# FT-Autonomous/ft_grandprix

Measured on AMD Instinct MI355X. Metric: env-steps/sec (4096 envs, 1080-ray LiDAR) at 1/2/4/8 MI355X; HBM roofline %, higher is better.
Workload: dtype f32 rays + f64 state

## Files before the change

ft_grandprix_amd/csrc/ftgp_api.hip:

```cpp
#include <dlfcn.h>
#include <math.h>
#include <cmath>
#include <stdarg.h>
#include <stdio.h>
#include <stdlib.h>
#include <string.h>

#include <algorithm>
#include <memory>
#include <string>
#include <type_traits>
#include <utility>
#include <vector>

#include <hip/hip_ext.h>
#include "ftgp_kernels.hip"

namespace {

thread_local char g_err[512] = "";

int fail(int code, const char* fmt, const char* a = "")
{
    snprintf(g_err, sizeof g_err, fmt, a);
    return code;
}

int failf(int code, const char* fmt, ...)
{
    va_list ap;
    va_start(ap, fmt);
    vsnprintf(g_err, sizeof g_err, fmt, ap);
    va_end(ap);
    return code;
}

int name_track(int code, int k)
{
    const std::string m(g_err);
// ... 366 lines not shown
        return FTGP_ERR_ARG;
    }
    if (sw.verbose)
        fprintf(stderr, "ftgp_create: %d cars x %d waves per workgroup, %d B of LDS (cap %d)\n", cpb, wpb, lds_layout(P, cpb, wpb), lds_cap);
    return 0;
}

void plan_fan(const FtgpConfig& cfg, std::vector<float>& ray, std::vector<double>& fan)
{
    const int R = cfg.n_rays;
    ray.assign((size_t)pad16(sizeof(float) * 2 * (size_t)R) / sizeof(float), 0.0f);
    fan.assign(2 * (size_t)R, 0.0);
    for (int j = 0; j < R; ++j) {
        const double phi = ((360.0 / (double)R) * (double)j - 90.0) * (M_PI / 180.0);
        fan[2 * (size_t)j] = cfg.fan_dirs ? cfg.fan_dirs[2 * (size_t)j] : sin(phi);
        fan[2 * (size_t)j + 1] = cfg.fan_dirs ? cfg.fan_dirs[2 * (size_t)j + 1] : -cos(phi);
        ray[2 * (size_t)j] = (float)fan[2 * (size_t)j]; ray[2 * (size_t)j + 1] = (float)fan[2 * (size_t)j + 1];
        if (!cfg.fan_dirs && R % 2 == 0 && j >= R / 2) {
            ray[2 * (size_t)j] = -ray[2 * (size_t)(j - R / 2)]; ray[2 * (size_t)j + 1] = -ray[2 * (size_t)(j - R / 2) + 1];
        }
    }
}

void plan_task_order(const FtgpConfig& cfg, const std::vector<float>& ray, const Switches& sw, DeviceParams& P)
{
    const int R = cfg.n_rays, halfR = R / 2;
    bool sym = R % 2 == 0 && !sw.no_pairs;
    for (int j = 0; sym && j < halfR; ++j)
        sym = ray[2 * (size_t)(j + halfR)] == -ray[2 * (size_t)j] && ray[2 * (size_t)(j + halfR) + 1] == -ray[2 * (size_t)j + 1] &&
              std::signbit(ray[2 * (size_t)(j + halfR)]) != std::signbit(ray[2 * (size_t)j]) && std::signbit(ray[2 * (size_t)(j + halfR) + 1]) != std::signbit(ray[2 * (size_t)j + 1]);
    std::vector<int> tasks;
    if (!sym) for (int j0 = 0; j0 < R; j0 += FTGP_WAVE) tasks.push_back(j0);
    else {
        int j0 = 0;
        for (; j0 + FTGP_WAVE <= halfR; j0 += FTGP_WAVE) tasks.push_back(j0 | (1 << 16));
        if (j0 < halfR) tasks.push_back(j0 | ((halfR - j0 <= FTGP_WAVE / 2 ? 2 : 1) << 16));
    }
    std::vector<std::pair<double, int>> key;
    for (int t : tasks) {
        const double mid = std::min((double)R - 1.0, (double)(t & 0xffff) + 31.5);
        key.push_back({ sw.group_order_plain ? 0.0 : -fabs(cos(2.0 * M_PI * mid / (double)R)), t });
    }
    std::stable_sort(key.begin(), key.end(), [](const std::pair<double, int>& a, const std::pair<double, int>& b) { return a.first < b.first; });
    const int tail = sw.pair_tail;
    std::vector<int> order;
    for (size_t k = 0; k < key.size(); ++k) {
        const int t = key[k].second;
        if ((t >> 16) == 1 && (int)(key.size() - k) <= tail) { order.push_back(t & 0xffff); order.push_back((t & 0xffff) + halfR); }
        else order.push_back(t);
    }
    P.tasks_per_car = (int)order.size();
    for (size_t k = 0; k < order.size(); ++k) P.group_order[k] = order[k];
    const double gamma = 32.0 * (2.0 * M_PI / (double)R) + 0.021;
// ... 7 lines not shown
    const int cpb = P.cars_per_block, ntasks = cpb * P.tasks_per_car, R = P.n_rays, halfR = R / 2;
    if (P.tasks_per_car > 256 || R > 0x4000) return fail(FTGP_ERR_ARG, "internal: the task table's fields are too narrow for this fan%s");
    tt.assign(2 * 4 * (size_t)ntasks, 0);
    auto wclass = [&](int first, int lim) {
        const int last = std::min(first + FTGP_WAVE, lim) - 1, lo = P.eighth, hi = R - P.eighth;
        if (last < lo || first >= hi || lo >= hi) return 0;
        return (first >= lo && last < hi) ? 1 : 2;
    };
    for (int g = 0; g < ntasks; ++g) {
        const int kidx = g / cpb, c = g % cpb, ent = P.group_order[kidx], j0 = ent & 0xffff, kind = ent >> 16;
        const int w0 = kind == 2 ? 2 : wclass(j0, kind == 1 ? halfR : R), w1 = kind == 1 ? wclass(j0 + halfR, R) : 0;
        const uint32_t plain = (uint32_t)j0 | (uint32_t)kind << 14 | (uint32_t)c << 16;
        int32_t* a = &tt[4 * (size_t)g];
        int32_t* b = &tt[4 * (size_t)(ntasks + g)];
        a[0] = (int32_t)(plain | (uint32_t)w0 << 20 | (uint32_t)w1 << 22 | (uint32_t)(j0 == 0 ? 1 : 0) << 24);
        b[0] = (int32_t)plain;
        a[1] = b[1] = c * (int)sizeof(LidarFrame) | kidx << 16;
        a[2] = b[2] = c * P.ranges_stride * 4;
        a[3] = b[3] = 4 * (c * P.win_floats + (P.eighth & 3) - P.eighth);
    }
    return 0;
}

void plan_window_table(const Switches& sw, const std::vector<int32_t>& tt, DeviceParams& P, std::vector<int32_t>& tw)
{
    const int cpb = P.cars_per_block, R = P.n_rays, halfR = R / 2;
    tw.clear();
    P.win_tasks_per_car = 0;
    if (sw.scan_every_step) {
        if (sw.verbose) fprintf(stderr, "ftgp_create: FTGP_SCAN_EVERY_STEP: every step of a launch sweeps and stores every ray\n");
        return;
    }
    auto live = [&](int j) { return j == 0 || (j >= P.eighth && j < R - P.eighth); };
    std::vector<std::pair<int, uint32_t>> list;
    for (int k = 0; k < P.tasks_per_car; ++k) {
        uint32_t x = (uint32_t)tt[4 * (size_t)k * cpb];
        const int j0 = x & 0x3fff, kind = (x >> 14) & 3;
        int n[2] = { 0, 0 }, l[2] = { 0, 0 };
        for (int lane = 0; lane < FTGP_WAVE; ++lane) {
            int j; bool mine;
            if (kind == 2) { j = j0 + (lane & 31) + (lane >= 32 ? halfR : 0); mine = (lane & 31) < halfR - j0; }
            else { j = j0 + lane; mine = j < (kind == 1 ? halfR : R); }
            if (!mine) continue;
            ++n[0]; l[0] += live(j) ? 1 : 0;
            if (kind == 1) { ++n[1]; l[1] += live(j + halfR) ? 1 : 0; }
        }
        if (l[0] + l[1] == 0) continue;
        if (kind == 1 && n[0] == FTGP_WAVE && (l[0] == 0 || l[1] == 0)) {
            if (l[0] == 0) { x = (uint32_t)(j0 + halfR) | ((x >> 22) & 3u) << 20 | 1u << 26; n[0] = n[1]; l[0] = l[1]; }
            else x &= ~(3u << 14 | 3u << 22);
            n[1] = l[1] = 0;
        }
        if (l[0] + l[1] < n[0] + n[1]) x |= 1u << 25;
        list.push_back({ k, x });
    }
    P.win_tasks_per_car = (int)list.size();
    const int ntasks = cpb * P.win_tasks_per_car;
    tw.assign(4 * (size_t)ntasks, 0);
    for (int g = 0; g < ntasks; ++g) {
        const int c = g % cpb, kidx = list[(size_t)(g / cpb)].first;
        const int32_t* a = &tt[4 * ((size_t)kidx * cpb + c)];
        int32_t* w = &tw[4 * (size_t)g];
        w[0] = (int32_t)(list[(size_t)(g / cpb)].second | (uint32_t)c << 16);
        w[1] = a[1]; w[2] = a[2]; w[3] = a[3];
    }
    if (sw.verbose) fprintf(stderr, "ftgp_create: %d of them on the window-only steps of a launch\n", P.win_tasks_per_car);
}

double track_diagonal(const FtgpTrack& t) { return hypot((double)t.width * t.px_size_x, (double)t.height * t.px_size_y); }

void plan_vehicle(const DeviceParams& P, double diag, const Switches& sw, std::vector<unsigned char>& img)
{
    const FtgpVehicle& v = P.veh;
    img.assign((size_t)pad16(sizeof(VehLds)), 0);
    VehLds vl; memset(&vl, 0, sizeof vl);
    vl.v = P.veh; for (int i = 0; i < 4; ++i) vl.wheel_load[i] = P.wheel_load[i];
    const double cx = std::max(fabs(v.box_xmin), fabs(v.box_xmax)), cy = std::max(fabs(v.box_ymin), fabs(v.box_ymax));
    const double rmax = std::max(sqrt(cx * cx + cy * cy), sqrt(v.lidar_x * v.lidar_x + v.lidar_y * v.lidar_y) + v.lidar_ring_radius);
    vl.cull_radius = (float)(1.1 * rmax);
    {
        const double r = v.lidar_ring_radius;
        const double need = r > 0.0 ? 5.0 * ldexp(1.0, -24) * diag * diag / (2.0 * r) : 0.0;
        const double have = std::min(std::min(v.lidar_x - r - v.box_xmin, v.box_xmax - (v.lidar_x + r)), std::min(v.lidar_y - r - v.box_ymin, v.box_ymax - (v.lidar_y + r)));
        vl.puck_in_box = (have >= need && !sw.puck_test) ? 1 : 0;
        if (sw.verbose)
            fprintf(stderr, "ftgp_create: inter-vehicle rays test %s (the puck lies %.4f inside the box, %.4f needed on a map of diagonal %.2f)\n",
                    vl.puck_in_box ? "the box only" : "the box and the puck's circle", have, need, diag);
// ... 66 lines not shown
    P.veh = cfg.vehicle;
    {
        const double wtot = v.mass * v.gravity;
        if (v.kind == FTGP_VEHICLE_TRICYCLE) {
            const double a_f = v.wheel_x[2], a_r = -0.5 * (v.wheel_x[0] + v.wheel_x[1]);
            P.wheel_load[0] = P.wheel_load[1] = 0.5 * (wtot * (a_f / (a_f + a_r)));
            P.wheel_load[2] = wtot * (a_r / (a_f + a_r)); P.wheel_load[3] = 0.0;
        } else {
            const double a_f = 0.5 * (v.wheel_x[0] + v.wheel_x[1]), a_r = -0.5 * (v.wheel_x[2] + v.wheel_x[3]);
            P.wheel_load[0] = P.wheel_load[1] = 0.5 * (wtot * (a_r / (a_f + a_r)));
            P.wheel_load[2] = P.wheel_load[3] = 0.5 * (wtot * (a_f / (a_f + a_r)));
        }
    }
    P.eighth = (int)((double)cfg.n_rays / 8.0);
    const double tiny = (double)1.401298464e-45f;
    P.cover_kmax = std::max(1, std::max(cover_count_host(0.24, P.rpp, tiny), cover_count_host(0.12, P.rpp, tiny)));
    P.win_floats = ((P.eighth & 3) + (cfg.n_rays - 2 * P.eighth) + 1 + 3) & ~3;
    P.n_cu = n_cu;
    if ((cfg.n_rays + FTGP_WAVE - 1) / FTGP_WAVE > FTGP_MAX_GROUPS) return fail(FTGP_ERR_ARG, "n_rays above 16384 is not supported%s");
    if (int rc = plan_shape(P, sw)) return rc;
    plan_fan(cfg, pl.ray, pl.fan);
    plan_task_order(cfg, pl.ray, sw, P);
    if (int rc = plan_task_table(P, pl.tasks)) return rc;
    plan_window_table(sw, pl.tasks, P, pl.tasks_win);
    {
        const size_t stride = (size_t)P.cover_kmax + 1, padded = (size_t)pad16(sizeof(float) * stride) / sizeof(float);
        pl.cover.assign(stride + padded + 4, 0.0f);
        build_cover_table(0.12, cfg.n_rays, P.cover_kmax, pl.cover.data());
        build_cover_table(0.06, cfg.n_rays, P.cover_kmax, pl.cover.data() + stride);
    }
    double diag = 0.0;
    pl.env_track.clear();
    for (int t = 0; t < n_tracks; ++t) {
        Plan::Track& k = pl.tracks[(size_t)t];
        k.P = P;
        plan_track_params(cfg, tracks[t], k.P);
        plan_track_tables(tracks[t], k.P, k.tab, k.spawn);
        k.clear.assign(2 * FTGP_PATH_POINTS, 0.0);
        ftgp_start_table(tracks[t], k.spawn.data(), k.clear.data());
        k.path.assign(tracks[t].path, tracks[t].path + 2 * FTGP_PATH_POINTS);
        diag = std::max(diag, track_diagonal(tracks[t]));
        pl.env_track.insert(pl.env_track.end(), (size_t)envs_per_track[t], t);
    }
    plan_vehicle(P, diag, sw, pl.veh);
    plan_workgroups(P.cars_per_block, cfg.cars_per_env, envs_per_track, n_tracks, sw.track_order, pl.wg);
    pl.n_wg = (int)pl.wg.size() / 4;
    if (sw.verbose)
// ... 2001 lines not shown
```

ft_grandprix_amd/csrc/ftgp_device.h:

```cpp
#pragma once
#include <hip/hip_runtime.h>
#include <stdint.h>
#include <stddef.h>
#include "../../include/ftgp.h"
#include "ftgp_march.h"
#include "ftgp_spawn.h"
#include "ftgp_net.h"
#include "ftgp_frame.h"
#include "ftgp_rival.h"

#define FTGP_WAVE 64
#define FTGP_MAX_GROUPS 256
#define FTGP_MAX_CARS_PER_BLOCK 16

struct alignas(16) CarCore {
    double x, y, qw, qz;
    double vx, vy, wz;
    double qs, qsd;
    double w[4];
    double u_speed, u_steer;
    double last_steer;
    double dist2;
    int32_t completion, laps, offset, n_times;
    int32_t good_start, finished, off_track, delta;
// ... 56 lines not shown
    const uint16_t* field;
    const uint32_t* bits;
    const uint32_t* nearbits;
    const void* veh_dev;
    const double* path;
    const double* spawn;
    const float* ray_dir;
    const float* cover_thr;
    CarState* cars;
    float* ranges;
    int64_t* steps;
    double* wg_metrics;
    unsigned int* wg_ticket;
    double* metrics_dev;
    double* metrics_host;
    double* wg_metrics_host;
    alignas(16) int32_t sector_tab[FTGP_SECTORS][4];
    FtgpVehicle veh;
    double wheel_load[4];
    const unsigned char* stage_img;
    int32_t stage_cover, reserved3;
    int32_t car_policy[FTGP_MAX_CARS_PER_BLOCK];
    int32_t group_order[FTGP_MAX_GROUPS];
    const int32_t* task_tab;
};

#define FTGP_PARAMS_BYTES ((sizeof(DeviceParams) + 15) & ~(size_t)15)

struct VehLds {
    FtgpVehicle v;
    double wheel_load[4];
    float cull_radius;
    int32_t puck_in_box;
    float box_xmin_f, box_xmax_f, box_ymin_f, box_ymax_f, lidar_x_f, lidar_y_f, ring_radius_f, pad_f;
};

enum { kDynMass = 0, kDynIzz, kDynFriction, kDynTireDamping, kDynThrottleKv, kDynThrottleForceLimit, kDynSteerKp, kDynSteerDamping, kDynWheelLoad };
template <class PP> __host__ __device__ inline double* dyn_table(PP p) { return reinterpret_cast<double*>(((uint64_t)p->dyn_table_hi << 32) | (uint64_t)p->dyn_table_lo); }
template <class PP> __host__ __device__ inline unsigned long long* dyn_rejected(PP p) { return reinterpret_cast<unsigned long long*>(dyn_table(p) + (size_t)p->n_cars * FTGP_DYN_RECORD); }
#define FTGP_DYN_BYTES(n_cars) ((size_t)(n_cars) * FTGP_DYN_RECORD * sizeof(double) + 16)
struct DynArgs {
    double base[FTGP_DYN_DOUBLES];
    double gravity, load_k[4];
    int32_t load_half[4];
    int32_t init, pad;
    const double* rows;
    const uint8_t* env_mask;
    const uint8_t* env_mask_or;
// ... 80 lines not shown
```

ft_grandprix_amd/csrc/ftgp_kernels.hip:

```cpp
#include "ftgp_device.h"

struct Force { double fx, fy, tz; };
struct Dyn { double x, y, qw, qz, vx, vy, wz, qs, qsd, w[4]; };
static_assert(sizeof(Dyn) == 104 && offsetof(CarCore, w) == offsetof(Dyn, w) && offsetof(CarCore, qsd) == offsetof(Dyn, qsd), "Dyn must mirror the head of CarCore");
#define FTGP_FORCE_TERMS 11

struct Lds {
    const VehLds* veh;
    const double* path;
    const float2* ray;
    CarCore* cars;
    LidarFrame* frame;
    PairCull* pairs;
    int64_t* steps;
    float* scan;
    int* list;
    int* pool;
    Force* terms;
    double* wnew;
    Dyn* next;
    Force* mates;
    const float* cover;
    unsigned char* mmask;
};
// ... 226 lines not shown
        "s_branch L_march_done_%=\n"
        "L_march_fix0_%=:\n\t"
        FTGP_MARCH_FIX("v_mov_b32_e32 %[f], 0\n\t", "%[mx]", "%[my]", "L_march_arrive0_%=")
        "L_march_fix1_%=:\n\t"
        FTGP_MARCH_FIX("v_cndmask_b32_e64 %[f], %[mx], %[my], %[stepx]\n\t", "%[nx]", "%[ny]", "L_march_arrive1_%=")
        "L_march_fix2_%=:\n\t"
        FTGP_MARCH_FIX("v_cndmask_b32_e64 %[f], %[nx], %[ny], %[stepx]\n\t", "%[mx]", "%[my]", "L_march_arrive2_%=")
        "L_march_done_%=:\n\t"
        "s_mov_b64 exec, %[ex0]\n\t"
        "v_min_f32_e32 %[s], %[a], %[b]"
        : [s] "=&v"(s), [w] "=&v"(w), [mx] "=&v"(mx), [my] "=&v"(my), [nx] "=&v"(nx), [ny] "=&v"(ny),
          [a] "=&v"(a), [b] "=&v"(b), [c] "=&v"(c), [d] "=&v"(d), [e] "=&v"(e), [f] "=&v"(f), [h] "=&v"(h), [i] "=&v"(i),
          [gu] "=&v"(gu), [gv] "=&v"(gv), [cx] "=&v"(cx), [cy] "=&v"(cy),
          [stepx] "=&s"(stepx), [sv] "=&s"(sv), [sq] "=&s"(sq), [ex0] "=&s"(ex0)
        : [pu] "v"(pu), [pv] "v"(pv), [ivx] "v"(ivx), [ivy] "v"(ivy), [du] "v"(du), [dv] "v"(dv),
          [base] "v"(base), [ax] "v"(ax), [ay] "v"(ay), [thr] "s"(thr), [field] "s"(field)
        : "vcc", "scc", "memory");
#undef FTGP_MARCH_BODY
#undef FTGP_MARCH_MOVE
#undef FTGP_MARCH_ARRIVE
#undef FTGP_MARCH_FIX
}

template <bool MULTI, bool WINDOW>
__device__ __forceinline__ void lidar_groups(const DeviceParams& P, ScalarParams G, const Lds& L, const LidarFrame* frames, const PairCull* pairs, const unsigned char* mmask,
                                             float* scan_rows, int* pool, int ncars_here, int ci0, bool scan_lds, bool second_half STAMP_ARG)
{
    typedef __attribute__((address_space(1))) float* global_f32;
    typedef __attribute__((address_space(1))) unsigned char* global_u8w;
    struct alignas(16) Task { int32_t x, y, z, w; };
    typedef const __attribute__((address_space(4))) Task* ScalarTasks;
    constexpr bool window_only = WINDOW;
    const int full_tasks = G->cars_per_block * G->tasks_per_car;
    const int R = G->n_rays, half = R >> 1, ntasks = window_only ? G->cars_per_block * G->win_tasks_per_car : full_tasks;
    const int W = G->width, H = G->height, fstride = G->fstride;
    const uint32_t plane256 = G->plane256;
    const int eighth = G->eighth, win_floats = G->win_floats;
    const float isx = G->inv_px_x_f, isy = G->inv_px_y_f, thr = 0.5f - G->snap_eps, nsf = G->slice_factor;
    const float r0 = sgpr(L.veh->ring_radius_f);
    const void* field = G->field;
    const ScalarTasks tasks = (ScalarTasks)G->task_tab + (window_only ? 2 * full_tasks : scan_lds ? 0 : full_tasks);
    const global_u8w ranges = (global_u8w)((global_f32)G->ranges + (size_t)ci0 * G->ranges_stride);
    const int mmask_stride = G->mmask_stride;
    const int lane = lane_here();
    const bool all_safe = sgpr(pool[4]) == 0;
    sweep_priority(second_half);
    for (;;) {
        STAMP(ta);
        int g = 0;
        if (lane == 0) g = atomicAdd(pool, 1);
        g = __builtin_amdgcn_readfirstlane(g);
        if (g >= ntasks) break;
        Task task; { const uint32_t gu = (uint32_t)g; task.x = tasks[gu].x; task.y = tasks[gu].y; task.z = tasks[gu].z; task.w = tasks[gu].w; }
        const int j0 = task.x & 0x3fff, kind = (task.x >> 14) & 3, c = (task.x >> 16) & 15;
        int j; bool mine;
        if (kind == 2) { j = j0 + (lane & 31) + (lane >= 32 ? half : 0); mine = (lane & 31) < half - j0; }
        else { j = j0 + lane; mine = j < (kind == 1 ? half : R); }
        mine = mine && c < ncars_here;
        bool first = mine;
        if (WINDOW && (task.x & (1 << 25))) {
            asm volatile("");
            first = mine && (j == 0 || (unsigned)(j - eighth) < (unsigned)(R - 2 * eighth));
            mine = first || (kind == 1 && mine && (unsigned)(j + half - eighth) < (unsigned)(R - 2 * eighth));
        }
        const LidarFrame* frame = reinterpret_cast<const LidarFrame*>(reinterpret_cast<const unsigned char*>(frames) + (task.y & 0xffff));
        FtgpRay ray;
        float du, dv, dxw, dyw, opu, opv;
        uint32_t sector;
        asm volatile("" : "=v"(du), "=v"(dv), "=v"(dxw), "=v"(dyw), "=v"(opu), "=v"(opv), "=v"(sector));
        auto finish = [&](bool active, int pass) {
            if (!active) return;
            uint32_t w;
            STAMP(tb);
            march_all(ray.s, w, opu, opv, ray.ivx, ray.ivy, du, dv, ray.base, ray.ax, ray.ay, thr, field);
            STAMP(tc); STAMP_ADD(10, tc - tb); STAMP_ADD(9, 1);
            float r = (w == 0u) ? fabsf(ray.s) : ray.result;
            if (MULTI && FTGP_DIAG_RUN_MATES) {
                const PairCull* mates = pairs + c * FTGP_PAIR_STRIDE;
                const int slot0 = sgpr(frame->slot0);
                const int kidx = task.y >> 16;
                uint32_t mm = (uint32_t)sgpr((int)mmask[c * mmask_stride + 2 * kidx + pass + (WINDOW ? (task.x >> 26) & 1 : 0)]);
                while (mm) {
                    const int k = __builtin_ctz(mm); mm &= mm - 1u;
                    const float4 q = *reinterpret_cast<const float4*>(mates + k);
                    const float al = fmaf(q.x, dxw, q.y * dyw);
                    if (al >= q.z) {
                        const float cull = L.veh->cull_radius;
                        if (r >= 0.0f && (al + r0) - cull > r) continue;
                        const float rc = ray_vs_car(L.veh, frames + slot0 + k, q.x, q.y, dxw, dyw);
                        if (rc < INFINITY && (r < 0.0f || rc < r)) r = rc;
                    }
                }
            }
            const uint32_t j4 = (uint32_t)j << 2;
            if (!window_only) *(global_f32)(ranges + (j4 + (uint32_t)task.z)) = r;
            const int wclass = (task.x >> (20 + 2 * pass)) & 3;
            if (wclass) {
                float* dst = reinterpret_cast<float*>(reinterpret_cast<unsigned char*>(scan_rows) + task.w + j4);
                if (wclass == 2) { asm volatile(""); dst = (unsigned)(j - eighth) < (unsigned)(R - 2 * eighth) ? dst : reinterpret_cast<float*>(pool + 6); }
                *dst = r;
            }
            if ((task.x & (1 << 24)) && pass == 0) {
                asm volatile("");
                if (j == 0) *reinterpret_cast<float*>(reinterpret_cast<unsigned char*>(scan_rows) + task.w + 4 * (win_floats - 1 - (eighth & 3) + eighth)) = r;
            }
        };
        if (mine) {
            const float4 f4 = *reinterpret_cast<const float4*>(frame);
            const float2 bd = L.ray[j];
            dxw = fmaf(f4.z, bd.x, -(f4.w * bd.y));
            dyw = fmaf(f4.w, bd.x, f4.z * bd.y);
            du = dxw * isx;
            dv = -(dyw * isy);
            const float pu = fmaf(du, -r0, f4.x);
            const float pv = fmaf(dv, -r0, f4.y);
            opu = pu; opv = pv;
            float ivx, ivy;
            rcp_abs2<true>(du, dv, ivx, ivy);
            ray.result = -1.0f;
            sector = ftgp_ray_sector(du, dv, ivx, ivy, nsf);
            ftgp_ray_place(ray, pu, pv, du, dv, ivx, ivy, sector, W, H, fstride, plane256, true, &P.sector_tab[0][0]);
            if (!all_safe) {
                ftgp_ray_park_if_outside(ray, pu, pv, W, H);
                ray.result = (f4.x == -INFINITY) ? 0.0f : -1.0f;
            }
        }
        STAMP(td); STAMP_ADD(8, td - ta);
        finish(first, 0);
        if (kind == 1) {
            if (WINDOW && (task.x & (1 << 25))) { asm volatile(""); mine = mine && (unsigned)(j + half - eighth) < (unsigned)(R - 2 * eighth); }
            if (mine) {
                j += half;
                const float2 f2 = *reinterpret_cast<const float2*>(frame);
                du = -du; dv = -dv; dxw = -dxw; dyw = -dyw;
                const float pu = fmaf(du, -r0, f2.x);
                const float pv = fmaf(dv, -r0, f2.y);
                opu = pu; opv = pv;
                ftgp_ray_place(ray, pu, pv, du, dv, ray.ivx, ray.ivy, sector ^ 3u, W, H, fstride, plane256, true, &P.sector_tab[0][0]);
                if (!all_safe) {
                    ftgp_ray_park_if_outside(ray, pu, pv, W, H);
                    ray.result = (f2.x == -INFINITY) ? 0.0f : -1.0f;
                }
            }
            finish(mine, 1);
        }
    }
}

__device__ __forceinline__ void march_fake(double& x, double& y, double& dist, int& bad, double dx, double dy, int W, int H, const double* dt)
{
    double n = 0.0, t, u;
    int xi, yi, a, b;
    uint64_t sq, ex0;
// ... 44 lines not shown
{
    typedef __attribute__((address_space(1))) float* global_f32;
    typedef __attribute__((address_space(1))) unsigned char* global_u8w;
    struct alignas(16) Task { int32_t x, y, z, w; };
    typedef const __attribute__((address_space(4))) Task* ScalarTasks;
    const int full_tasks = G->cars_per_block * G->tasks_per_car;
    const int R = G->n_rays, half = R >> 1, ntasks = window_only ? G->cars_per_block * G->win_tasks_per_car : full_tasks;
    const int W = G->width, H = G->height;
    const int eighth = G->eighth, win_floats = G->win_floats;
    const double s = G->map_size;
    const double* dt = G->edt;
    const double* __restrict__ fan = G->fan_dirs;
    const ScalarTasks tasks = (ScalarTasks)G->task_tab + (window_only ? 2 * full_tasks : scan_lds ? 0 : full_tasks);
    const global_u8w ranges = (global_u8w)((global_f32)G->ranges + (size_t)ci0 * G->ranges_stride);
    const int lane = lane_here();
    for (;;) {
        int g = 0;
        if (lane == 0) g = atomicAdd(pool, 1);
        g = __builtin_amdgcn_readfirstlane(g);
        if (g >= ntasks) break;
        Task task; { const uint32_t gu = (uint32_t)g; task.x = tasks[gu].x; task.y = tasks[gu].y; task.z = tasks[gu].z; task.w = tasks[gu].w; }
        const int j0 = task.x & 0x3fff, kind = (task.x >> 14) & 3, c = (task.x >> 16) & 15;
        int j; bool mine;
        if (kind == 2) { j = j0 + (lane & 31) + (lane >= 32 ? half : 0); mine = (lane & 31) < half - j0; }
        else { j = j0 + lane; mine = j < (kind == 1 ? half : R); }
        mine = mine && c < ncars_here;
        const LidarFrame* f = reinterpret_cast<const LidarFrame*>(reinterpret_cast<const unsigned char*>(frames) + (task.y & 0xffff));
        for (int pass = 0; pass < (kind == 1 ? 2 : 1); ++pass, j += half) {
            if (!mine || ((task.x & (1 << 25)) && j != 0 && (unsigned)(j - eighth) >= (unsigned)(R - 2 * eighth))) continue;
            float r = 0.0f;
            if (!f->finished) {
                const double ch = f->x, sh = f->y;
                const double bx = fan[2 * j], by = fan[2 * j + 1];
                const double dxw = ch * bx - sh * by, dyw = sh * bx + ch * by;
                double x = f->lcx, y = f->lcy, distance = 0.0;
                int bad = 0;
                march_fake(x, y, distance, bad, dxw, -dyw, W, H, dt);
                r = bad ? -1.0f : (float)((distance / (double)W) * s);
            }
            const uint32_t j4 = (uint32_t)j << 2;
            if (!window_only) *(global_f32)(ranges + (j4 + (uint32_t)task.z)) = r;
            const int wclass = (task.x >> (20 + 2 * pass)) & 3;
            if (wclass) {
                float* dst = reinterpret_cast<float*>(reinterpret_cast<unsigned char*>(scan_rows) + task.w + j4);
                if (wclass == 2) { asm volatile(""); dst = (unsigned)(j - eighth) < (unsigned)(R - 2 * eighth) ? dst : reinterpret_cast<float*>(pool + 6); }
                *dst = r;
            }
            if ((task.x & (1 << 24)) && pass == 0) {
                asm volatile("");
                if (j == 0) *reinterpret_cast<float*>(reinterpret_cast<unsigned char*>(scan_rows) + task.w + 4 * (win_floats - 1 - (eighth & 3) + eighth)) = r;
            }
        }
// ... 234 lines not shown
__device__ __forceinline__ void pair_cull_write(const LidarFrame* frames, PairCull* pairs, int c, int k, int cars_per_env, float cull, float r0)
{
    const LidarFrame* me = frames + c;
    const int mate = me->slot0 + k;
    PairCull p; p.bx = 0.0f; p.by = 0.0f; p.t = INFINITY; p.pad = 0.0f;
    if (k < cars_per_env && mate != c && !me->finished && !frames[mate].finished) {
        p.bx = (float)(frames[mate].x - me->lcx); p.by = (float)(frames[mate].y - me->lcy);
        const float d2 = p.bx * p.bx + p.by * p.by, close = 2.0f * cull + r0;
        p.t = d2 <= close * close ? -INFINITY : sqrtf(d2 - cull * cull) * 0.9999f;
    }
    pairs[c * FTGP_PAIR_STRIDE + k] = p;
}

typedef const __attribute__((address_space(4))) int32_t* ScalarInts;
__device__ __forceinline__ void mate_masks(const LidarFrame* frames, const PairCull* pairs, unsigned char* mmask, int mmask_stride, ScalarInts order,
                                           const float2* __restrict__ ray_tab, int R, int tasks, int cars_per_env, float cull, float cg, float sg,
                                           int ncars_here, int first, int step)
{
    const int slots = 2 * tasks;
    for (int idx = first; idx < ncars_here * slots; idx += step) {
        const int c = idx / slots, s = idx - c * slots;
        const int ent = order[s >> 1], j0 = ent & 0xffff, kind = ent >> 16;
        uint32_t m = 0;
        if (kind == 2 || cg < -1.0f) m = (s & 1) ? 0u : 0xffu;
        else if (!(s & 1) || kind == 1) {
            const int jc = min(j0 + 32, (kind == 1 ? (R >> 1) : R) - 1);
            const float2 bd = ray_tab[jc];
            const LidarFrame* me = frames + c;
            float dxw = fmaf(me->chf, bd.x, -(me->shf * bd.y)), dyw = fmaf(me->shf, bd.x, me->chf * bd.y);
            if (s & 1) { dxw = -dxw; dyw = -dyw; }
            for (int k = 0; k < cars_per_env; ++k) {
                const float4 q = *reinterpret_cast<const float4*>(pairs + c * FTGP_PAIR_STRIDE + k);
                const float al = fmaf(q.x, dxw, q.y * dyw);
                if (al >= fmaf(cg, q.z, -(sg * cull)) - 1e-4f) m |= 1u << k;
            }
        }
        mmask[c * mmask_stride + s] = (unsigned char)m;
    }
}

template <int QUAD_PERM>
__device__ __forceinline__ void quad_argmin_step(double& best, int& idx)
{
    const int lo = __double2loint(best), hi = __double2hiint(best);
    const double ob = __hiloint2double(__builtin_amdgcn_update_dpp(hi, hi, QUAD_PERM, 0xf, 0xf, false), __builtin_amdgcn_update_dpp(lo, lo, QUAD_PERM, 0xf, 0xf, false));
    const int oi = __builtin_amdgcn_update_dpp(idx, idx, QUAD_PERM, 0xf, 0xf, false);
    if (ob < best || (ob == best && oi < idx)) { best = ob; idx = oi; }
}

template <bool MULTI, bool DYN>
__device__ __forceinline__ void dynamics_lanes(const DeviceParams& P, const Lds& L, LidarFrame* next_frames, PairCull* next_pairs, unsigned char* next_mmask, ScalarInts order,
                                               int* unsafe_next, int ncars_here, int ci0, const double* dyn)
{
    const int lane = lane_here();
    const int c = lane >> 2, r = lane & 3;
    const bool on = c < ncars_here;
    CarCore* st = L.cars + (on ? c : 0);
    Force* terms = L.terms + (on ? c : 0) * FTGP_FORCE_TERMS;
    const FtgpVehicle& v = L.veh->v;
    const bool finished = st->finished != 0;
    SUBSTAMP_BEGIN();
    {
        const double* mine = dyn + (on ? c : 0) * FTGP_DYN_RECORD;
        const double qw = st->qw, qz = st->qz;
        const double ch = 1.0 - 2.0 * (qz * qz), sh = 2.0 * (qw * qz);
        const double vx = st->vx, vy = st->vy, wz = st->wz;
        const double q = st->qs;
        const double c1 = (r == 0) ? 0.375 : -0.375;
        const double q4 = q * 0.0722656, t3 = (r == 0) ? -q4 : q4;
        const double steer = q * (1.0 + q * (c1 + q * (0.140625 + t3)));
        const bool tri = sgpr(v.kind) == FTGP_VEHICLE_TRICYCLE;
        const double ang = (!tri && r < 2) ? steer : 0.0;
        const double cwi = spec_cos(ang), swi = spec_sin(ang);
        double torque;
// ... 157 lines not shown
        quad_argmin_step<0x4E>(best, idx);
    }
    SUBSTAMP(5);
    if (upd) {
        Race rc; race_load(rc, upd_st);
        progress_update(P, rc, L.steps[upd_c], idx, best, P.cars[ci0 + upd_c].times, &upd_st->start);
        race_store(rc, upd_st);
    }
    wave_lds_sync();
    SUBSTAMP(6);
    bool safe = true;
    if (on && r == 0) safe = frame_write(P, v, st, next_frames + c, c);
    const bool any_unsafe = __any(!safe);
    if (lane == 0) *unsafe_next = any_unsafe;
    SUBSTAMP(7);
    if (MULTI) {
        wave_lds_sync();
        const float cull = L.veh->cull_radius, r0f = (float)v.lidar_ring_radius;
        if (on) {
            pair_cull_write(next_frames, next_pairs, c, r, P.cars_per_env, cull, r0f);
            pair_cull_write(next_frames, next_pairs, c, r + 4, P.cars_per_env, cull, r0f);
        }
        wave_lds_sync();
        mate_masks(next_frames, next_pairs, next_mmask, P.mmask_stride, order, L.ray, P.n_rays, P.tasks_per_car, P.cars_per_env, cull, P.group_cg, P.group_sg, ncars_here, lane, FTGP_WAVE);
    }
}

__device__ __forceinline__ int wave_inclusive_sum(int x)
{
    const int s1 = __builtin_amdgcn_update_dpp(0, x, 0x111, 0xf, 0xf, true);
    const int s2 = __builtin_amdgcn_update_dpp(0, x, 0x112, 0xf, 0xf, true);
    const int s3 = __builtin_amdgcn_update_dpp(0, x, 0x113, 0xf, 0xf, true);
    int v = x + s1 + s2 + s3;
    v += __builtin_amdgcn_update_dpp(0, v, 0x114, 0xf, 0xe, true);
    v += __builtin_amdgcn_update_dpp(0, v, 0x118, 0xf, 0xc, true);
    v += __builtin_amdgcn_update_dpp(0, v, 0x142, 0xa, 0xf, true);
    v += __builtin_amdgcn_update_dpp(0, v, 0x143, 0xc, 0xf, true);
    return v;
}

#define FTGP_DPP_REDUCE(op) \
    "s_nop 1\n\t" op " %0, %0, %0 row_shr:1 row_mask:0xf bank_mask:0xf\n\t" \
    "s_nop 1\n\t" op " %0, %0, %0 row_shr:2 row_mask:0xf bank_mask:0xf\n\t" \
    "s_nop 1\n\t" op " %0, %0, %0 row_shr:4 row_mask:0xf bank_mask:0xf\n\t" \
    "s_nop 1\n\t" op " %0, %0, %0 row_shr:8 row_mask:0xf bank_mask:0xf\n\t" \
    "s_nop 1\n\t" op " %0, %0, %0 row_bcast:15 row_mask:0xa bank_mask:0xf\n\t" \
    "s_nop 1\n\t" op " %0, %0, %0 row_bcast:31 row_mask:0xc bank_mask:0xf\n\t" \
// ... 615 lines not shown
            for (int c = 0; c < ncars_here; ++c)
                L.scan[(cpb + c) * win_floats + scan_window_first(eighth) + j] = P.ranges[(size_t)(ci0 + c) * P.ranges_stride + eighth + j];
        }
        if ((int)threadIdx.x < ncars_here) L.scan[(cpb + (int)threadIdx.x) * win_floats + win_floats - 1] = P.ranges[(size_t)(ci0 + (int)threadIdx.x) * P.ranges_stride];
    }
    for (int c = wave; c < ncars_here; c += nwaves) {
        const int ci = ci0 + c;
        if (lane < (int)(sizeof(CarCore) / 4))
            reinterpret_cast<uint32_t*>(L.cars + c)[lane] = reinterpret_cast<const uint32_t*>(static_cast<const CarCore*>(&P.cars[ci]))[lane];
        if (lane == 0) L.steps[c] = P.steps[ci / P.cars_per_env];
        wave_lds_sync();
        if (lane == 0 && !frame_write(P, L.veh->v, L.cars + c, L.frame + c, c)) atomicOr(L.pool + 4, 1);
    }
    if (DYN) {
        const double* src = dyn_table(scalar_view(Pt)) + (size_t)ci0 * FTGP_DYN_RECORD;
        double* dst = reinterpret_cast<double*>(lds + P.lds_bytes);
        for (int i = (int)threadIdx.x; i < ncars_here * FTGP_DYN_RECORD; i += (int)blockDim.x) dst[i] = src[i];
    }
    if (MULTI) {
        __syncthreads();
        for (int idx = (int)threadIdx.x; idx < ncars_here * FTGP_PAIR_STRIDE; idx += (int)blockDim.x)
            pair_cull_write(L.frame, L.pairs, idx / FTGP_PAIR_STRIDE, idx % FTGP_PAIR_STRIDE, P.cars_per_env, L.veh->cull_radius, (float)L.veh->v.lidar_ring_radius);
        __syncthreads();
        if (wave == 0)
            mate_masks(L.frame, L.pairs, L.mmask, P.mmask_stride, &scalar_view(Pt)->group_order[0], L.ray, P.n_rays, P.tasks_per_car, P.cars_per_env, L.veh->cull_radius, P.group_cg, P.group_sg,
                       ncars_here, lane_here(), FTGP_WAVE);
    }
    }
    __syncthreads();

    STAMP_DECLARE();
    for (int it = 0; it < n_steps; ++it) {
        STAMP(t0);
        const int par = it & 1;
        if (wave < ncars_here) {
            const ScalarParams G = scalar_view(Pt);
            const LdsOffsets off = lds_offsets(G);
            const DeviceParams& P = *reinterpret_cast<const DeviceParams*>(lds + off.params);
            const Lds L = lds_view(off, lds);
            const int win_floats = G->win_floats;
            LidarFrame* next_frames = L.frame + (par ^ 1) * cpb;
            float* scan_prev = L.scan + (par ^ 1) * cpb * win_floats;
            if (FTGP_DIAG_PRIO) __builtin_amdgcn_s_setprio(3);
            for (int c = wave; c < ncars_here; c += nwaves) {
                if constexpr (NET) {
                    const int pol = policy == FTGP_POLICY_PER_CAR ? G->car_policy[c] : policy;
                    if (is_net_policy(pol)) policy_apply_net(net_table(G), pol - FTGP_POLICY_NET0, scan_prev + c * win_floats, G->eighth, L.cars + c,
                                                            [&] { const int cpe = G->cars_per_env, sl = c % cpe; return NetEnv{ L.path, L.cars + (c - sl), (int)sizeof(CarCore), sl, cpe }; },
                                                            [&] { return (ci0 + c) / G->cars_per_env; });
                    else if (policy == FTGP_POLICY_PER_CAR)
                        policy_apply(P, driver_shape(G), pol, scan_prev + c * win_floats, L.cars + c, ci0 + c, L.steps[c], L.list + wave * FTGP_WAVE,
                                     L.cover + (pol == FTGP_POLICY_FAST ? (G->stage_cover >> 2) : 0));
                }
                else if (ROSTER && policy == FTGP_POLICY_PER_CAR) {
                    const int pol = G->car_policy[c];
                    policy_apply(P, driver_shape(G), pol, scan_prev + c * win_floats, L.cars + c, ci0 + c, L.steps[c], L.list + wave * FTGP_WAVE,
                                 L.cover + (pol == FTGP_POLICY_FAST ? (G->stage_cover >> 2) : 0));
                }
                else if (policy != FTGP_POLICY_HOST) policy_apply(P, driver_shape(G), policy, scan_prev + c * win_floats, L.cars + c, ci0 + c, L.steps[c], L.list + wave * FTGP_WAVE, L.cover);
                wave_lds_sync();
                int n = 0;
                if (lane_here() == 0) n = __hip_atomic_fetch_add(L.pool + 2 + par, 1, __ATOMIC_ACQ_REL, __HIP_MEMORY_SCOPE_WORKGROUP);
                n = __builtin_amdgcn_readfirstlane(n);
                __builtin_amdgcn_fence(__ATOMIC_ACQUIRE, "workgroup");
                STAMP(t1); STAMP_ADD(0, t1 - t0);
                if (n == ncars_here - 1) {
                    if (lane_here() == 0) { L.pool[par ^ 1] = 0; L.pool[2 + (par ^ 1)] = 0; }
                    if (FTGP_DIAG_RUN_K1)
                        dynamics_lanes<MULTI, DYN>(P, L, next_frames, L.pairs + (par ^ 1) * cpb * FTGP_PAIR_STRIDE, L.mmask + (par ^ 1) * cpb * G->mmask_stride, &G->group_order[0],
                                                   L.pool + 4 + (par ^ 1), ncars_here, ci0, DYN ? reinterpret_cast<const double*>(lds + opaque(G->lds_bytes)) : nullptr);
                    STAMP(t2); STAMP_ADD(2, t2 - t1); STAMP_ADD(7, 1);
                }
            }
            if (FTGP_DIAG_PRIO) __builtin_amdgcn_s_setprio(0);
        }
        STAMP(t3);
        if (FTGP_DIAG_RUN_K2) {
            const ScalarParams G = scalar_view(Pt);
            const LdsOffsets off = lds_offsets(G);
            const DeviceParams& P = *reinterpret_cast<const DeviceParams*>(lds + off.params);
            const Lds L = lds_view(off, lds);
            const bool window_only = need_scan && it != n_steps - 1 && G->win_tasks_per_car != 0;
            if (FAKE) lidar_fake(G, L.frame + par * cpb, L.scan + par * cpb * G->win_floats, L.pool + par, ncars_here, ci0, need_scan, window_only);
            else if (window_only)
                lidar_groups<MULTI, true>(P, G, L, L.frame + par * cpb, L.pairs + par * cpb * FTGP_PAIR_STRIDE, L.mmask + par * cpb * G->mmask_stride, L.scan + par * cpb * G->win_floats,
                                          L.pool + par, ncars_here, ci0, true, second_half STAMP_PASS);
            else
                lidar_groups<MULTI, false>(P, G, L, L.frame + par * cpb, L.pairs + par * cpb * FTGP_PAIR_STRIDE, L.mmask + par * cpb * G->mmask_stride, L.scan + par * cpb * G->win_floats,
                                           L.pool + par, ncars_here, ci0, need_scan, second_half STAMP_PASS);
        }
        STAMP(t4);
        __syncthreads();
// ... 1128 lines not shown
```

Baseline: 247.2 million.

## Repack window-only lidar tasks into dense groups with gathered leftover runs

Window-only steps now get their own task set, built by cutting the live ray window into full 64-lane pairs and singles plus gather tasks that pack the leftover fragments (ray 0, zone edges) into full waves through per-lane offset runs. This replaces partially-live groups that masked dead lanes at run time, so fewer waves are launched and the per-lane liveness checks disappear. Mate masks are now computed against a separate win_group_order on steps whose next step is window-only. The cost is a new task kind with a small lookup per lane, more complex host planning, and a layout dependency between group_order and win_group_order.

Measured after the change: 264.2 million (median of 6 runs). 1.07x the previous value.

```diff
diff --git a/ft_grandprix_amd/csrc/ftgp_api.hip b/ft_grandprix_amd/csrc/ftgp_api.hip
--- a/ft_grandprix_amd/csrc/ftgp_api.hip
+++ b/ft_grandprix_amd/csrc/ftgp_api.hip
@@ -15,6 +15,7 @@
 
 #include <hip/hip_ext.h>
 #include "ftgp_kernels.hip"
+#include "ftgp_window_cut.h"
 
 namespace {
 
@@ -427,13 +428,20 @@
     }
 }
 
-void plan_task_order(const FtgpConfig& cfg, const std::vector<float>& ray, const Switches& sw, DeviceParams& P)
-{
-    const int R = cfg.n_rays, halfR = R / 2;
+bool fan_allows_pairs(const std::vector<float>& ray, int R, const Switches& sw)
+{
+    const int halfR = R / 2;
     bool sym = R % 2 == 0 && !sw.no_pairs;
     for (int j = 0; sym && j < halfR; ++j)
         sym = ray[2 * (size_t)(j + halfR)] == -ray[2 * (size_t)j] && ray[2 * (size_t)(j + halfR) + 1] == -ray[2 * (size_t)j + 1] &&
               std::signbit(ray[2 * (size_t)(j + halfR)]) != std::signbit(ray[2 * (size_t)j]) && std::signbit(ray[2 * (size_t)(j + halfR) + 1]) != std::signbit(ray[2 * (size_t)j + 1]);
+    return sym;
+}
+
+void plan_task_order(const FtgpConfig& cfg, const std::vector<float>& ray, const Switches& sw, DeviceParams& P)
+{
+    const int R = cfg.n_rays, halfR = R / 2;
+    const bool sym = fan_allows_pairs(ray, R, sw);
     std::vector<int> tasks;
     if (!sym) for (int j0 = 0; j0 < R; j0 += FTGP_WAVE) tasks.push_back(j0);
     else {
@@ -487,47 +495,67 @@
     return 0;
 }
 
-void plan_window_table(const Switches& sw, const std::vector<int32_t>& tt, DeviceParams& P, std::vector<int32_t>& tw)
+void plan_window_table(const Switches& sw, const std::vector<float>& ray, const std::vector<int32_t>& tt, DeviceParams& P, std::vector<int32_t>& tw)
 {
     const int cpb = P.cars_per_block, R = P.n_rays, halfR = R / 2;
     tw.clear();
     P.win_tasks_per_car = 0;
+    for (int k = 0; k < FTGP_MAX_GROUPS; ++k) P.win_group_order[k] = 0;
     if (sw.scan_every_step) {
         if (sw.verbose) fprintf(stderr, "ftgp_create: FTGP_SCAN_EVERY_STEP: every step of a launch sweeps and stores every ray\n");
         return;
     }
-    auto live = [&](int j) { return j == 0 || (j >= P.eighth && j < R - P.eighth); };
-    std::vector<std::pair<int, uint32_t>> list;
-    for (int k = 0; k < P.tasks_per_car; ++k) {
-        uint32_t x = (uint32_t)tt[4 * (size_t)k * cpb];
-        const int j0 = x & 0x3fff, kind = (x >> 14) & 3;
-        int n[2] = { 0, 0 }, l[2] = { 0, 0 };
-        for (int lane = 0; lane < FTGP_WAVE; ++lane) {
-            int j; bool mine;
-            if (kind == 2) { j = j0 + (lane & 31) + (lane >= 32 ? halfR : 0); mine = (lane & 31) < halfR - j0; }
-            else { j = j0 + lane; mine = j < (kind == 1 ? halfR : R); }
-            if (!mine) continue;
-            ++n[0]; l[0] += live(j) ? 1 : 0;
-            if (kind == 1) { ++n[1]; l[1] += live(j + halfR) ? 1 : 0; }
+    const bool dead = P.eighth > 0;
+    const FtgpWindowCut cut = ftgp_window_cut(R, P.eighth, fan_allows_pairs(ray, R, sw));
+    auto along = [&](double j) { return fabs(cos(2.0 * M_PI * j / (double)R)); };
+    struct Ent { double key; int ent, gather; };
+    std::vector<Ent> key;
+    for (int j0 : cut.pairs) key.push_back({ -along(j0 + 31.5), j0 | 1 << 16, -1 });
+    for (int j0 : cut.singles) key.push_back({ -along(j0 + 31.5), j0, -1 });
+    for (size_t q = 0; q < cut.gathers.size(); ++q) {
+        double sum = 0.0; int lanes = 0;
+        for (const FtgpWindowCut::Run& r : cut.gathers[q]) { for (int j = r.first; j < r.first + r.second; ++j) sum += along(j); lanes += r.second; }
+        key.push_back({ -sum / lanes, lanes | (int)q << 7 | 3 << 16, (int)q });
+    }
+    if (sw.group_order_plain) for (Ent& k : key) k.key = 0.0;
+    std::stable_sort(key.begin(), key.end(), [](const Ent& a, const Ent& b) { return a.key < b.key; });
+    std::vector<int> order;
+    for (int tail = std::max(0, sw.pair_tail); ; --tail) {
+        order.clear();
+        for (size_t k = 0; k < key.size(); ++k) {
+            const int t = key[k].ent;
+            if ((t >> 16) == 1 && (int)(key.size() - k) <= tail) { order.push_back(t & 0xffff); order.push_back((t & 0xffff) + halfR); }
+            else order.push_back(t);
         }
-        if (l[0] + l[1] == 0) continue;
-        if (kind == 1 && n[0] == FTGP_WAVE && (l[0] == 0 || l[1] == 0)) {
-            if (l[0] == 0) { x = (uint32_t)(j0 + halfR) | ((x >> 22) & 3u) << 20 | 1u << 26; n[0] = n[1]; l[0] = l[1]; }
-            else x &= ~(3u << 14 | 3u << 22);
-            n[1] = l[1] = 0;
+        if ((int)order.size() <= P.tasks_per_car || tail == 0) break;
+    }
+    if (!dead || (int)order.size() > P.tasks_per_car || cut.gathers.size() > 127) {
+        P.win_tasks_per_car = P.tasks_per_car;
+        for (int k = 0; k < P.tasks_per_car; ++k) P.win_group_order[k] = P.group_order[k];
+        tw.assign(tt.begin(), tt.begin() + 4 * (size_t)cpb * P.tasks_per_car);
+        if (sw.verbose) fprintf(stderr, "ftgp_create: %d of them on the window-only steps of a launch\n", P.win_tasks_per_car);
+        return;
+    }
+    P.win_tasks_per_car = (int)order.size();
+    for (size_t k = 0; k < order.size(); ++k) P.win_group_order[k] = order[k];
+    const int ntasks = cpb * P.win_tasks_per_car;
+    tw.assign(4 * ((size_t)ntasks + cut.gathers.size()), 0);
+    for (int g = 0; g < ntasks; ++g) {
+        const int kidx = g / cpb, c = g % cpb, ent = order[(size_t)kidx], kind = ent >> 16;
+        const int32_t* a = &tt[4 * (size_t)c];
+        int32_t* w = &tw[4 * (size_t)g];
+        bool zero = false;
+        if (kind == 3) for (const FtgpWindowCut::Run& r : cut.gathers[(size_t)((ent >> 7) & 127)]) zero = zero || r.first == 0;
+        w[0] = (int32_t)((uint32_t)(ent & 0x3fff) | (uint32_t)kind << 14 | (uint32_t)c << 16 | (kind == 3 ? 2u : 1u) << 20 | (kind == 1 ? 1u : 0u) << 22 | (zero ? 1u : 0u) << 24);
+        w[1] = (a[1] & 0xffff) | kidx << 16; w[2] = a[2]; w[3] = a[3];
+    }
+    for (size_t q = 0; q < cut.gathers.size(); ++q) {
+        int32_t* w = &tw[4 * ((size_t)ntasks + q)];
+        int lane = 0;
+        for (size_t k = 0; k < 4; ++k) {
+            if (k < cut.gathers[q].size()) { w[k] = (int32_t)((uint32_t)((cut.gathers[q][k].first - lane) & 0xffff) | (uint32_t)lane << 16); lane += cut.gathers[q][k].second; }
+            else w[k] = (int32_t)(64u << 16);
         }
-        if (l[0] + l[1] < n[0] + n[1]) x |= 1u << 25;
-        list.push_back({ k, x });
-    }
-    P.win_tasks_per_car = (int)list.size();
-    const int ntasks = cpb * P.win_tasks_per_car;
-    tw.assign(4 * (size_t)ntasks, 0);
-    for (int g = 0; g < ntasks; ++g) {
-        const int c = g % cpb, kidx = list[(size_t)(g / cpb)].first;
-        const int32_t* a = &tt[4 * ((size_t)kidx * cpb + c)];
-        int32_t* w = &tw[4 * (size_t)g];
-        w[0] = (int32_t)(list[(size_t)(g / cpb)].second | (uint32_t)c << 16);
-        w[1] = a[1]; w[2] = a[2]; w[3] = a[3];
     }
     if (sw.verbose) fprintf(stderr, "ftgp_create: %d of them on the window-only steps of a launch\n", P.win_tasks_per_car);
 }
@@ -640,7 +668,7 @@
     plan_fan(cfg, pl.ray, pl.fan);
     plan_task_order(cfg, pl.ray, sw, P);
     if (int rc = plan_task_table(P, pl.tasks)) return rc;
-    plan_window_table(sw, pl.tasks, P, pl.tasks_win);
+    plan_window_table(sw, pl.ray, pl.tasks, P, pl.tasks_win);
     {
         const size_t stride = (size_t)P.cover_kmax + 1, padded = (size_t)pad16(sizeof(float) * stride) / sizeof(float);
         pl.cover.assign(stride + padded + 4, 0.0f);
diff --git a/ft_grandprix_amd/csrc/ftgp_device.h b/ft_grandprix_amd/csrc/ftgp_device.h
--- a/ft_grandprix_amd/csrc/ftgp_device.h
+++ b/ft_grandprix_amd/csrc/ftgp_device.h
@@ -102,8 +102,11 @@
     int32_t stage_cover, reserved3;
     int32_t car_policy[FTGP_MAX_CARS_PER_BLOCK];
     int32_t group_order[FTGP_MAX_GROUPS];
+    int32_t win_group_order[FTGP_MAX_GROUPS];
     const int32_t* task_tab;
 };
+
+static_assert(offsetof(DeviceParams, win_group_order) == offsetof(DeviceParams, group_order) + sizeof(int32_t) * FTGP_MAX_GROUPS, "win_group_order lies right behind group_order (dynamics_lanes)");
 
 #define FTGP_PARAMS_BYTES ((sizeof(DeviceParams) + 15) & ~(size_t)15)
 
diff --git a/ft_grandprix_amd/csrc/ftgp_kernels.hip b/ft_grandprix_amd/csrc/ftgp_kernels.hip
--- a/ft_grandprix_amd/csrc/ftgp_kernels.hip
+++ b/ft_grandprix_amd/csrc/ftgp_kernels.hip
@@ -272,6 +272,19 @@
 #undef FTGP_MARCH_FIX
 }
 
+template <class ScalarTasksT>
+__device__ __forceinline__ void gather_lanes(ScalarTasksT gathers, int field, int lane, int& j, bool& mine)
+{
+    const uint32_t q = (uint32_t)field >> 7;
+    const int r0 = gathers[q].x, r1 = gathers[q].y, r2 = gathers[q].z, r3 = gathers[q].w;
+    int d = (int16_t)r0;
+    if (lane >= (r1 >> 16)) d = (int16_t)r1;
+    if (lane >= (r2 >> 16)) d = (int16_t)r2;
+    if (lane >= (r3 >> 16)) d = (int16_t)r3;
+    j = lane + d;
+    mine = lane < (field & 127);
+}
+
 template <bool MULTI, bool WINDOW>
 __device__ __forceinline__ void lidar_groups(const DeviceParams& P, ScalarParams G, const Lds& L, const LidarFrame* frames, const PairCull* pairs, const unsigned char* mmask,
                                              float* scan_rows, int* pool, int ncars_here, int ci0, bool scan_lds, bool second_half STAMP_ARG)
@@ -304,15 +317,10 @@
         Task task; { const uint32_t gu = (uint32_t)g; task.x = tasks[gu].x; task.y = tasks[gu].y; task.z = tasks[gu].z; task.w = tasks[gu].w; }
         const int j0 = task.x & 0x3fff, kind = (task.x >> 14) & 3, c = (task.x >> 16) & 15;
         int j; bool mine;
-        if (kind == 2) { j = j0 + (lane & 31) + (lane >= 32 ? half : 0); mine = (lane & 31) < half - j0; }
+        if (WINDOW && kind == 3) { asm volatile(""); gather_lanes(tasks + ntasks, j0, lane, j, mine); }
+        else if (kind == 2) { j = j0 + (lane & 31) + (lane >= 32 ? half : 0); mine = (lane & 31) < half - j0; }
         else { j = j0 + lane; mine = j < (kind == 1 ? half : R); }
         mine = mine && c < ncars_here;
-        bool first = mine;
-        if (WINDOW && (task.x & (1 << 25))) {
-            asm volatile("");
-            first = mine && (j == 0 || (unsigned)(j - eighth) < (unsigned)(R - 2 * eighth));
-            mine = first || (kind == 1 && mine && (unsigned)(j + half - eighth) < (unsigned)(R - 2 * eighth));
-        }
         const LidarFrame* frame = reinterpret_cast<const LidarFrame*>(reinterpret_cast<const unsigned char*>(frames) + (task.y & 0xffff));
         FtgpRay ray;
         float du, dv, dxw, dyw, opu, opv;
@@ -329,7 +337,7 @@
                 const PairCull* mates = pairs + c * FTGP_PAIR_STRIDE;
                 const int slot0 = sgpr(frame->slot0);
                 const int kidx = task.y >> 16;
-                uint32_t mm = (uint32_t)sgpr((int)mmask[c * mmask_stride + 2 * kidx + pass + (WINDOW ? (task.x >> 26) & 1 : 0)]);
+                uint32_t mm = (uint32_t)sgpr((int)mmask[c * mmask_stride + 2 * kidx + pass]);
                 while (mm) {
                     const int k = __builtin_ctz(mm); mm &= mm - 1u;
                     const float4 q = *reinterpret_cast<const float4*>(mates + k);
@@ -376,9 +384,8 @@
             }
         }
         STAMP(td); STAMP_ADD(8, td - ta);
-        finish(first, 0);
+        finish(mine, 0);
         if (kind == 1) {
-            if (WINDOW && (task.x & (1 << 25))) { asm volatile(""); mine = mine && (unsigned)(j + half - eighth) < (unsigned)(R - 2 * eighth); }
             if (mine) {
                 j += half;
                 const float2 f2 = *reinterpret_cast<const float2*>(frame);
@@ -469,12 +476,13 @@
         Task task; { const uint32_t gu = (uint32_t)g; task.x = tasks[gu].x; task.y = tasks[gu].y; task.z = tasks[gu].z; task.w = tasks[gu].w; }
         const int j0 = task.x & 0x3fff, kind = (task.x >> 14) & 3, c = (task.x >> 16) & 15;
         int j; bool mine;
-        if (kind == 2) { j = j0 + (lane & 31) + (lane >= 32 ? half : 0); mine = (lane & 31) < half - j0; }
+        if (kind == 3) gather_lanes(tasks + ntasks, j0, lane, j, mine);
+        else if (kind == 2) { j = j0 + (lane & 31) + (lane >= 32 ? half : 0); mine = (lane & 31) < half - j0; }
         else { j = j0 + lane; mine = j < (kind == 1 ? half : R); }
         mine = mine && c < ncars_here;
         const LidarFrame* f = reinterpret_cast<const LidarFrame*>(reinterpret_cast<const unsigned char*>(frames) + (task.y & 0xffff));
         for (int pass = 0; pass < (kind == 1 ? 2 : 1); ++pass, j += half) {
-            if (!mine || ((task.x & (1 << 25)) && j != 0 && (unsigned)(j - eighth) >= (unsigned)(R - 2 * eighth))) continue;
+            if (!mine) continue;
             float r = 0.0f;
             if (!f->finished) {
                 const double ch = f->x, sh = f->y;
@@ -755,7 +763,7 @@
         const int c = idx / slots, s = idx - c * slots;
         const int ent = order[s >> 1], j0 = ent & 0xffff, kind = ent >> 16;
         uint32_t m = 0;
-        if (kind == 2 || cg < -1.0f) m = (s & 1) ? 0u : 0xffu;
+        if (kind >= 2 || cg < -1.0f) m = (s & 1) ? 0u : 0xffu;
         else if (!(s & 1) || kind == 1) {
             const int jc = min(j0 + 32, (kind == 1 ? (R >> 1) : R) - 1);
             const float2 bd = ray_tab[jc];
@@ -782,7 +790,7 @@
 }
 
 template <bool MULTI, bool DYN>
-__device__ __forceinline__ void dynamics_lanes(const DeviceParams& P, const Lds& L, LidarFrame* next_frames, PairCull* next_pairs, unsigned char* next_mmask, ScalarInts order,
+__device__ __forceinline__ void dynamics_lanes(const DeviceParams& P, const Lds& L, LidarFrame* next_frames, PairCull* next_pairs, unsigned char* next_mmask, ScalarInts order, bool win_next,
                                                int* unsafe_next, int ncars_here, int ci0, const double* dyn)
 {
     const int lane = lane_here();
@@ -986,7 +994,7 @@
             pair_cull_write(next_frames, next_pairs, c, r + 4, P.cars_per_env, cull, r0f);
         }
         wave_lds_sync();
-        mate_masks(next_frames, next_pairs, next_mmask, P.mmask_stride, order, L.ray, P.n_rays, P.tasks_per_car, P.cars_per_env, cull, P.group_cg, P.group_sg, ncars_here, lane, FTGP_WAVE);
+        mate_masks(next_frames, next_pairs, next_mmask, P.mmask_stride, win_next ? order + FTGP_MAX_GROUPS : order, L.ray, P.n_rays, win_next ? P.win_tasks_per_car : P.tasks_per_car, P.cars_per_env, cull, P.group_cg, P.group_sg, ncars_here, lane, FTGP_WAVE);
     }
 }
 
@@ -1648,9 +1656,11 @@
         for (int idx = (int)threadIdx.x; idx < ncars_here * FTGP_PAIR_STRIDE; idx += (int)blockDim.x)
             pair_cull_write(L.frame, L.pairs, idx / FTGP_PAIR_STRIDE, idx % FTGP_PAIR_STRIDE, P.cars_per_env, L.veh->cull_radius, (float)L.veh->v.lidar_ring_radius);
         __syncthreads();
-        if (wave == 0)
-            mate_masks(L.frame, L.pairs, L.mmask, P.mmask_stride, &scalar_view(Pt)->group_order[0], L.ray, P.n_rays, P.tasks_per_car, P.cars_per_env, L.veh->cull_radius, P.group_cg, P.group_sg,
-                       ncars_here, lane_here(), FTGP_WAVE);
+        if (wave == 0) {
+            const bool win0 = need_scan && n_steps != 1 && P.win_tasks_per_car != 0;
+            mate_masks(L.frame, L.pairs, L.mmask, P.mmask_stride, win0 ? &scalar_view(Pt)->win_group_order[0] : &scalar_view(Pt)->group_order[0], L.ray, P.n_rays,
+                       win0 ? P.win_tasks_per_car : P.tasks_per_car, P.cars_per_env, L.veh->cull_radius, P.group_cg, P.group_sg, ncars_here, lane_here(), FTGP_WAVE);
+        }
     }
     }
     __syncthreads();
@@ -1692,8 +1702,9 @@
                 STAMP(t1); STAMP_ADD(0, t1 - t0);
                 if (n == ncars_here - 1) {
                     if (lane_here() == 0) { L.pool[par ^ 1] = 0; L.pool[2 + (par ^ 1)] = 0; }
+                    const bool win_next = need_scan && it + 1 != n_steps - 1 && G->win_tasks_per_car != 0;
                     if (FTGP_DIAG_RUN_K1)
-                        dynamics_lanes<MULTI, DYN>(P, L, next_frames, L.pairs + (par ^ 1) * cpb * FTGP_PAIR_STRIDE, L.mmask + (par ^ 1) * cpb * G->mmask_stride, &G->group_order[0],
+                        dynamics_lanes<MULTI, DYN>(P, L, next_frames, L.pairs + (par ^ 1) * cpb * FTGP_PAIR_STRIDE, L.mmask + (par ^ 1) * cpb * G->mmask_stride, &G->group_order[0], win_next,
                                                    L.pool + 4 + (par ^ 1), ncars_here, ci0, DYN ? reinterpret_cast<const double*>(lds + opaque(G->lds_bytes)) : nullptr);
                     STAMP(t2); STAMP_ADD(2, t2 - t1); STAMP_ADD(7, 1);
                 }
diff --git a/ft_grandprix_amd/csrc/ftgp_window_cut.h b/ft_grandprix_amd/csrc/ftgp_window_cut.h
--- /dev/null
+++ b/ft_grandprix_amd/csrc/ftgp_window_cut.h
@@ -0,0 +1,42 @@
+#pragma once
+#include <utility>
+#include <vector>
+
+struct FtgpWindowCut {
+    typedef std::pair<int, int> Run;
+    std::vector<int> pairs;
+    std::vector<int> singles;
+    std::vector<std::vector<Run>> gathers;
+};
+
+inline FtgpWindowCut ftgp_window_cut(int R, int e, bool pairs_allowed, bool side_low = true, bool cone_low = true)
+{
+    FtgpWindowCut cut;
+    std::vector<FtgpWindowCut::Run> rest;
+    rest.push_back({ 0, 1 });
+    const int h = R / 2, lo = e, hi = R - e;
+    auto zone = [&](int a, int b, bool low, std::vector<int>& groups, bool opposite) {
+        const int n = b - a, whole = n / 64, left = n - 64 * whole, first = low ? a + left : a;
+        for (int k = 0; k < whole; ++k) groups.push_back(first + 64 * k);
+        if (left) {
+            const int r0 = low ? a : b - left;
+            rest.push_back({ r0, left });
+            if (opposite) rest.push_back({ r0 + h, left });
+        }
+    };
+    if (1 + (hi - lo) <= 64) { if (hi > lo) rest.push_back({ lo, hi - lo }); }
+    else if (pairs_allowed) {
+        zone(lo, h - e, side_low, cut.pairs, true);
+        zone(h - e, h + e, cone_low, cut.singles, false);
+    }
+    else zone(lo, hi, cone_low, cut.singles, false);
+    std::vector<FtgpWindowCut::Run> cur; int lanes = 0;
+    for (FtgpWindowCut::Run r : rest)
+        while (r.second > 0) {
+            const int n = r.second < 64 - lanes ? r.second : 64 - lanes;
+            cur.push_back({ r.first, n }); lanes += n; r.first += n; r.second -= n;
+            if (lanes == 64) { cut.gathers.push_back(cur); cur.clear(); lanes = 0; }
+        }
+    if (!cur.empty()) cut.gathers.push_back(cur);
+    return cut;
+}
```
